# Agzs/BlockMaze

Hardware: AMD Instinct MI355X
Metric: Groth16 proofs/sec (send circuit, alt_bn128) (higher is better)
Workload: dtype u32 limbs (254-bit Fq/Fr Montgomery; all MSM accumulations, the H query's weighted bucket sum and the transforms' tiles on nine 29-bit limbs)

## Files before the change

### __graft_entry__.py

```python
import os, subprocess, sys

ROOT = os.path.dirname(os.path.abspath(__file__))
if ROOT not in sys.path:
    sys.path.insert(0, ROOT)

def build():
    subprocess.check_call(["make", "-C", os.path.join(ROOT, "blockmaze_amd", "csrc"), "-j8"])
    subprocess.check_call(["make", "-s", "-C", os.path.join(ROOT, "blockmaze_amd", "csrc"), "-j8", "tsan"])
    subprocess.check_call(["make", "-C", os.path.join(ROOT, "oracle"), "oracle"])
    if os.path.isdir("/root/reference/libsnark-vnt"):
        subprocess.check_call(["make", "-C", os.path.join(ROOT, "oracle"), "-j8", "ref"])
    import blockmaze_amd
    from blockmaze_amd import engine
    engine.lib()

def smoke():
    import numpy as np
    sys.path.insert(0, os.path.join(ROOT, "tests"))
    from blockmaze_amd import engine as e
    from oracle import pyoracle as o
    from r1cs_util import random_r1cs
    e.init()
    n = 2000; g = o.SplitMix64(1); P = o.g1_consecutive(g.field(), n); K = o.to_arr([g.field() for _ in range(n)])
    got = o.g1_from(e.msm(1, P, K))[0]; assert got == o.msm_g1(P, K), "MSM mismatch vs oracle"
    cs, z = random_r1cs(3, 3, 200, 300); dev = e.R1cs(3, 200, 300, cs.rowptr, cs.col, cs.coeff)
    assert np.array_equal(dev.witness_map(z), o.witness_map(cs, z)), "witness map mismatch vs oracle"
    import json
    d = os.path.join(ROOT, "tests", "golden", "groth16_small"); meta = json.load(open(os.path.join(d, "meta.json"))); z = o.load_witness(os.path.join(d, "wit.bin"))
    p = e.Prover(os.path.join(d, "pk.txt")); proof = p.prove(z, int(meta["r"], 16), int(meta["s"], 16)); p.close()
    assert proof == meta["proof"], "proof bytes differ from the reference prover's"
    assert e.verify(os.path.join(d, "vk.txt"), proof, o.from_arr(z[:meta["n_inputs"]]))
    print("smoke ok: MSM, witness map and a Groth16 proof on", e.lib().zkgpu_version().decode(), "match the oracle")

if __name__ == "__main__":
    build()
```

### blockmaze_amd/csrc/capi_engine.cpp

```cpp
#include <cstring>
#include <memory>
#include <mutex>
#include <string>
#include <vector>
#include "../../include/zkgpu.h"
#include "gpu.hpp"

namespace zk {
void probe_field(int field, int op, const uint8_t *a, const uint8_t *b, uint8_t *out, size_t n);
void probe_fq2(int op, const uint8_t *a, const uint8_t *b, uint8_t *out, size_t n);
void probe_group(int group, int op, const uint8_t *a, const uint8_t *b, uint8_t *out, size_t n);
void probe_field29(int field, int op, const uint32_t *a, const uint32_t *b, const uint32_t *c, const uint32_t *d, uint32_t *out, size_t n);
void probe_point29(int op, const uint32_t *a, const uint32_t *b, uint32_t *out, uint32_t *flags, size_t n);
}
using namespace zk;
using namespace zk::host;

static thread_local std::string g_err;
void zkgpu_set_error(const std::string &s) { g_err = s; }
std::mutex g_gpu_mutex;

template <class Fn> static int guarded(Fn fn) {
  try { if (!gpu_available()) { g_err = "no HIP device visible; libzkgpu has no CPU fallback"; return ZKGPU_ERR_NO_DEVICE; }
        std::lock_guard<std::mutex> lk(g_gpu_mutex); return fn(); }
// ... 66 lines not shown
    }
    else {
      std::vector<G2AffineRaw> raw(n ? n : 1);
      for (size_t i = 0; i < n; i++) g2_to_raw(points + 128 * i, raw[i]);
      m->g2.reset(new MsmG2(raw.data(), n, c, (filter_ones & 1) != 0, true, (filter_ones & 2) != 0));
    }
    m->scalars = DevBuf<Fe32>(n ? n : 1); h = m.release(); return ZKGPU_OK; });
  return rc == ZKGPU_OK ? h : nullptr;
}
int zkgpu_msm_set_scalars(zkgpu_msm *h, const uint8_t *scalars, size_t n) { return guarded([&] { if (!h || n != h->n) { g_err = "scalar count";
    return ZKGPU_ERR_ARG; }
  if (n) { h->scalars.upload((const Fe32 *)scalars, n); fr_to_mont_dev(h->scalars.get(), n); gpu_sync(); } return ZKGPU_OK; }); }
int zkgpu_msm_run(zkgpu_msm *h, uint8_t *out) { return guarded([&] { if (!h) return ZKGPU_ERR_ARG;
  if (h->group == 1) { h->g1->run(h->scalars.get(), nullptr); g1_out(h->g1->result(), out); } else { h->g2->run(h->scalars.get(), nullptr);
      g2_out(h->g2->result(), out); } return ZKGPU_OK; }); }
void zkgpu_msm_destroy(zkgpu_msm *h) { guarded([&] { delete h; return ZKGPU_OK; }); }
static int msm_oneshot(int group, const uint8_t *points, const uint8_t *scalars, size_t n, int c, int fo, uint8_t *out) {
  zkgpu_msm *h = zkgpu_msm_create(group, points, n, c, fo);
  if (!h) return ZKGPU_ERR_RUNTIME;
  int rc = zkgpu_msm_set_scalars(h, scalars, n);
  if (rc == ZKGPU_OK) rc = zkgpu_msm_run(h, out);
  zkgpu_msm_destroy(h);
  return rc;
}
int zkgpu_msm_g1(const uint8_t *points, const uint8_t *scalars, size_t n, int c, int fo, uint8_t out[64]) {
  return msm_oneshot(1, points, scalars, n, c, fo, out);
}
int zkgpu_msm_g2(const uint8_t *points, const uint8_t *scalars, size_t n, int c, int fo, uint8_t out[128]) {
  return msm_oneshot(2, points, scalars, n, c, fo, out);
}

size_t zkgpu_domain_size(size_t min_size) {
  if (min_size <= 1) return 0; size_t lg = 0; while (((size_t)1 << lg) < min_size) lg++; if (min_size == ((size_t)1 << lg)) return lg <= 28 ? min_size : 0;
  size_t big = (size_t)1 << (lg - 1), small = min_size - big, rs = 1;
  while (rs < small) rs <<= 1;
  size_t m = (small == rs) ? min_size : big + rs;
  return lg <= 28 ? m : 0;
}
int zkgpu_domain_transform(size_t min_size, int op, uint8_t *data) { return guarded([&] { Domain d(min_size); size_t m = d.m(); DevBuf<Fe32> buf(m);
    buf.upload((const Fe32 *)data, m); fr_to_mont_dev(buf.get(), m);
  switch (op) {
    case 0: d.fft(buf.get(), 1, m);
    break;
    case 1: d.ifft(buf.get(), 1, m);
    break;
    case 2: d.coset_fft(buf.get(), 1, m);
    break;
    case 3: d.icoset_fft(buf.get(), 1, m);
    break;
    default: g_err = "op";
    return ZKGPU_ERR_ARG;
  }
  fr_from_mont_dev(buf.get(), m); buf.download((Fe32 *)data, m); return ZKGPU_OK; }); }

struct zkgpu_r1cs { R1csHost host; std::unique_ptr<R1csDev> dev; std::unique_ptr<Domain> dom; };
zkgpu_r1cs *zkgpu_r1cs_create(size_t n_inputs, size_t n_vars, size_t n_cons, const uint32_t *const rowptr[3], const uint32_t *const col[3],
    const uint8_t *const coeff[3]) {
  zkgpu_r1cs *out = nullptr;
  guarded([&] { std::unique_ptr<zkgpu_r1cs> h(new zkgpu_r1cs); h->host.n_inputs = n_inputs; h->host.n_vars = n_vars; h->host.n_cons = n_cons;
    for (int m = 0; m < 3; m++) {
      size_t nnz = rowptr[m][n_cons];
      h->host.rowptr[m].assign(rowptr[m], rowptr[m] + n_cons + 1);
      h->host.col[m].assign(col[m], col[m] + nnz);
      h->host.coeff[m].resize(nnz);
      if (nnz) memcpy(h->host.coeff[m].data(), coeff[m], 32 * nnz);
    }
    h->dev.reset(new R1csDev(h->host)); h->dom.reset(new Domain(n_cons + n_inputs + 1)); out = h.release(); return ZKGPU_OK; });
  return out;
}
void zkgpu_r1cs_destroy(zkgpu_r1cs *cs) { guarded([&] { delete cs; return ZKGPU_OK; }); }
int zkgpu_witness_map(zkgpu_r1cs *cs, const uint8_t *z, uint8_t *h_out) { return guarded([&] { if (!cs) return ZKGPU_ERR_ARG;
  size_t m = cs->dom->m(), nv = cs->host.n_vars; std::vector<Fe32> zz(nv + 1); memset(&zz[0], 0, 32); zz[0].l[0] = 1; if (nv) memcpy(&zz[1], z, 32 * nv);
  DevBuf<Fe32> zd(nv + 1), abc(3 * m); zd.upload(zz.data(), nv + 1); fr_to_mont_dev(zd.get(), nv + 1);
  cs->dev->eval(zd.get(), abc.get(), m);
  if (!cs->dev->satisfied(abc.get(), m)) {
    g_err = "assignment does not satisfy the constraint system";
    return ZKGPU_ERR_UNSATISFIED;
  }
  cs->dom->ifft(abc.get(), 3, m);
  cs->dom->coset_fft(abc.get(), 3, m);
  cs->dom->qap_pointwise(abc.get(), abc.get() + m, abc.get() + 2 * m);
  cs->dom->icoset_fft(abc.get(), 1, m);
  fr_from_mont_dev(abc.get(), m); abc.download((Fe32 *)h_out, m); memset(h_out + 32 * m, 0, 32); return ZKGPU_OK; }); }
}
```

### blockmaze_amd/csrc/gpu.hip

```cpp
#include <hip/hip_runtime.h>
#include <cstdio>
#include <cstdlib>
#include <chrono>
#include <cstring>
#include <map>
#include <vector>
#include <algorithm>
#include <mutex>
#include <atomic>
#include <mutex>
#include "gpu_internal.hpp"
#include "ntt.cuh"
#include "ecntt.cuh"

__attribute__((constructor(101))) static void zkgpu_load_time_environment() { setenv("GPU_MAX_HW_QUEUES", "16", 0); }

namespace zk {

constexpr int MAX_LANES_PER_DEVICE = 31, MAX_LANES = 1 + 8 * 28;
static uint8_t g_lane_claimed[MAX_LANES];
static std::atomic<GpuContext *> g_lanes[MAX_LANES];
static std::atomic<int> g_lane_slot[MAX_LANES];
static std::mutex g_lane_mutex;
static thread_local int t_lane = 0;
// ... 639 lines not shown
  if (cs.n_vars > cs.n_inputs) dl.upload(L, cs.n_vars - cs.n_inputs);
  DevBuf<uint8_t> b0(m * sizeof(XYZZ<Fq>)), b1(m * sizeof(XYZZ<Fq>)); XYZZ<Fq> *X = (XYZZ<Fq> *)b0.get(), *Y = (XYZZ<Fq> *)b1.get();
  auto stages = [&](XYZZ<Fq> *x, const Fe32 *tw, int lg) {
    for (int st = lg; st >= 1; st--) hipLaunchKernelGGL(k_ecntt_stage, dim3(cdiv(((size_t)1 << lg) / 2, 64)), dim3(64), 0, s, x, (const Fr *)tw, lg, st);
  };
  auto columns = [&](const XYZZ<Fq> *U, int lg) { hipLaunchKernelGGL(k_fold_c_columns, dim3(cdiv(n_all, 64)), dim3(64), 0, s, d_colptr.get(), d_rowidx.get(),
      d_kind.get(), (const Fr *)d_coef.get(), U, lg,
                     (const Affine<Fq> *)dl.get(), (uint32_t)cs.n_inputs, (uint32_t)n_all, (Affine<Fq> *)dout.get()); };
  if (!d.step) {
    HFr zinv; { Fe32 z; d.zinv.download(&z, 1); memcpy(zinv.l, &z, 32); } Fr fz; memcpy(&fz, zinv.l, 32);
    std::vector<Fe32> gm = geometric_table(m, HFr::from_u64(m).inv(), fr_coset_gen());
    DevBuf<Fe32> d_gm(m);
    d_gm.upload(gm.data(), m);
    hipLaunchKernelGGL(k_ecntt_scale_const, dim3(cdiv(m, 64)), dim3(64), 0, s, (const Affine<Fq> *)dp.get(), fz, (uint32_t)m, X);
    stages(X, d.big->tw.get(), logm);
    hipLaunchKernelGGL(k_ecntt_permute_scale, dim3(cdiv(m, 64)), dim3(64), 0, s, (const XYZZ<Fq> *)X, (const Fr *)d_gm.get(), logm, Y);
    stages(Y, d.big->itw.get(), logm);
    columns(Y, logm);
  } else {
    const int lb = d.big->logn, ls = d.small->logn;
    hipLaunchKernelGGL(k_ecntt_scale_table, dim3(cdiv(m, 64)), dim3(64), 0, s, (const Affine<Fq> *)dp.get(), (const Fr *)d.zinv.get(), (uint32_t)m, X);
    stages(X, d.big->tw.get(), lb);
    stages(X + d.B, d.small->tw.get(), ls);
    hipLaunchKernelGGL(k_ecntt_step_fwd_T, dim3(cdiv(d.B, 64)), dim3(64), 0, s, (const XYZZ<Fq> *)X, (const XYZZ<Fq> *)(X + d.B), lb, ls,
        (const Fr *)d.wpow.get(), (const Fr *)d.coset_fwd.get(), Y);
    HFr ib = HFr::from_u64(d.B).inv(), is = HFr::from_u64(d.S).inv(), hib = d.half * ib, his = d.half * is;
    Fr f_hib, f_ib, f_his;
    memcpy(&f_hib, hib.l, 32);
    memcpy(&f_ib, ib.l, 32);
    memcpy(&f_his, his.l, 32);
    hipLaunchKernelGGL(k_ecntt_step_pre, dim3(cdiv(m, 64)), dim3(64), 0, s, (const XYZZ<Fq> *)Y, X, (const Fr *)d.wpow.get(), (const Fr *)d.winvpow.get(),
        f_hib, f_ib, f_his, (uint32_t)d.B, (uint32_t)d.S);
    stages(X, d.big->itw.get(), lb); stages(X + d.B, d.small->itw.get(), ls);
    hipLaunchKernelGGL(k_ecntt_unpermute, dim3(cdiv(d.B, 64)), dim3(64), 0, s, (const XYZZ<Fq> *)X, lb, Y);
    hipLaunchKernelGGL(k_ecntt_unpermute, dim3(cdiv(d.S, 64)), dim3(64), 0, s, (const XYZZ<Fq> *)(X + d.B), ls, Y + d.B);
    columns(Y, 0);
  }
  HIP_CHECK(hipGetLastError()); dout.download(out, n_all);
}
const Fe32 *Domain::zinv_dev() const { return impl->zinv.get(); }
bool Domain::zinv_is_table() const { return impl->step; }
void Domain::qap_pointwise(Fe32 *a, const Fe32 *b, const Fe32 *c) {
  hipLaunchKernelGGL(k_qap_pointwise, dim3(cdiv(impl->m, 256)), dim3(256), 0, gpu().stream, (Fr *)a, (const Fr *)b, (const Fr *)c,
      (const Fr *)impl->zinv.get(), impl->step ? 1 : 0, (uint32_t)impl->m);
}

void expand_witness_dev(const uint8_t *packed, size_t words, const Fe32 &one_value, int canon, size_t n, Fe32 *out, uint8_t *tags, uint32_t *other_vars) {
  const uint64_t *ones = (const uint64_t *)packed, *other = ones + words, *third = other + words; const size_t nbm = canon == 2 ? 3 : 2;
  const uint32_t *off = (const uint32_t *)(ones + nbm * words); const Fr *vals = (const Fr *)(packed + expand_values_offset(words, canon));
  Fr one; memcpy(&one, &one_value, 32);
  hipLaunchKernelGGL(k_expand_witness, dim3(cdiv(n, 256)), dim3(256), 0, gpu().stream, ones, other,
      canon == 0 ? (const uint64_t *)nullptr : canon == 1 ? other : third, off, vals, one, zk_with_prio(n, ZKP_EXPAND), (Fr *)out, tags, other_vars);
}
void classify_witness_dev(const Fe32 *z, size_t n, uint8_t *tags, uint32_t *other_vars, uint32_t *counters, int parity) {
  Fr one; memcpy(&one, FrParams::R1, 32);
  hipLaunchKernelGGL(k_classify_witness, dim3(cdiv(n, 256 * CLASSIFY_PER_LANE)), dim3(256), 0, gpu().stream, (const Fr *)z, one, zk_with_prio(n, ZKP_EXPAND), tags, other_vars,
      counters + (parity & 1), counters + ((parity & 1) ^ 1));
}
void expand_board_dev(const uint8_t *board_tags, size_t n, const uint32_t *cand, const Fe32 *cand_vals, size_t n_cand, Fe32 *z, uint8_t *tags, uint32_t *other_vars,
    uint32_t *counters, int parity, bool vals_by_var) {
  Fr one; memcpy(&one, FrParams::R1, 32); const unsigned tb = cdiv(n, 256);
  hipLaunchKernelGGL(k_expand_board, dim3(tb + cdiv(n_cand, 256)), dim3(256), 0, gpu().stream, board_tags, zk_with_prio(n, ZKP_EXPAND), tb, cand, (const Fr *)cand_vals,
      (uint32_t)n_cand | (vals_by_var ? 0x80000000u : 0u), one, (Fr *)z, tags, other_vars, counters + (parity & 1), counters + ((parity & 1) ^ 1));
}
void *gpu_host_register(void *p, size_t bytes) {
  if (!p || !bytes) return nullptr; gpu();
  if (hipHostRegister(p, bytes, hipHostRegisterPortable | hipHostRegisterMapped) != hipSuccess) { (void)hipGetLastError(); return nullptr; }
  void *d = nullptr; if (hipHostGetDevicePointer(&d, p, 0) != hipSuccess || !d) { (void)hipGetLastError(); hipHostUnregister(p); return nullptr; }
  return d;
}
void gpu_host_unregister(void *p) { if (p) { (void)hipHostUnregister(p); (void)hipGetLastError(); } }
static std::atomic<uint64_t> g_general_path_repeats{0}, g_queries_without_tables{0};
uint64_t queries_without_tables() { return g_queries_without_tables.load(std::memory_order_relaxed); }
void note_query_without_tables() { g_queries_without_tables.fetch_add(1, std::memory_order_relaxed); }
uint64_t general_path_repeats() { return g_general_path_repeats.load(std::memory_order_relaxed); }
void note_general_path_repeat() { g_general_path_repeats.fetch_add(1, std::memory_order_relaxed); }
void merge_equal_columns_dev(Fe32 *z, uint8_t *tags, const uint32_t *grp_ptr, const uint32_t *grp_mem, size_t n_groups) {
  if (n_groups) hipLaunchKernelGGL(k_merge_equal_columns, dim3(cdiv(n_groups, 64)), dim3(64), 0, gpu().stream, (Fr *)z, tags, grp_ptr, grp_mem, (uint32_t)n_groups);
}
void fr_to_mont_dev(Fe32 *a, size_t n) { if (n) hipLaunchKernelGGL(k_fr_to_mont, dim3(cdiv(n, 256)), dim3(256), 0, gpu().stream, (Fr *)a, (uint32_t)n); }
void fr_from_mont_dev(Fe32 *a, size_t n) { if (n) hipLaunchKernelGGL(k_fr_from_mont, dim3(cdiv(n, 256)), dim3(256), 0, gpu().stream, (Fr *)a, (uint32_t)n); }

struct R1csArrays { size_t n_inputs, n_vars, n_cons; DevBuf<uint32_t> rowptr[3], col[3], cid[3], long_rows[3]; size_t n_long[3] = {0, 0, 0}; DevBuf<Fe32> ctab;
    DevBuf<uint32_t> long_any; size_t n_long_any = 0; };
struct R1csDev::Impl {
  std::shared_ptr<R1csArrays> a;
  size_t &n_inputs, &n_vars, &n_cons;
  DevBuf<uint32_t> (&rowptr)[3], (&col)[3], (&cid)[3], (&long_rows)[3];
  size_t (&n_long)[3];
  DevBuf<Fe32> &ctab;
  DevBuf<uint32_t> &long_any;
  size_t &n_long_any;
  DevBuf<uint32_t> flag;
  uint32_t *h_flag = nullptr;
  uint32_t *h_fail = nullptr, *d_fail = nullptr, seq = 0;
  explicit Impl(std::shared_ptr<R1csArrays> aa) : a(aa), n_inputs(a->n_inputs), n_vars(a->n_vars), n_cons(a->n_cons), rowptr(a->rowptr), col(a->col),
      cid(a->cid), long_rows(a->long_rows), n_long(a->n_long), ctab(a->ctab), long_any(a->long_any), n_long_any(a->n_long_any) {
  }
  void own_words() {
    flag = DevBuf<uint32_t>(1);
    HIP_CHECK(hipHostMalloc((void **)&h_flag, 4));
    HIP_CHECK(hipHostMalloc((void **)&h_fail, 8, hipHostMallocMapped));
    h_fail[0] = 0; h_fail[1] = 0;
    HIP_CHECK(hipHostGetDevicePointer((void **)&d_fail, h_fail, 0));
  }
  ~Impl() { if (h_flag) hipHostFree(h_flag); if (h_fail) hipHostFree(h_fail); }
};
R1csDev::R1csDev(const R1csDev &peer) : impl(new Impl(peer.impl->a)) { impl->own_words(); }
R1csDev::R1csDev(const R1csHost &h) : impl(new Impl(std::make_shared<R1csArrays>())) {
  Impl &d = *impl; d.n_inputs = h.n_inputs; d.n_vars = h.n_vars; d.n_cons = h.n_cons;
  std::vector<Fe32> tab(2); { HFr one = HFr::one(), m1 = one.neg(); memcpy(&tab[0], one.l, 32); memcpy(&tab[1], m1.l, 32); }
  struct Key { uint32_t l[8]; bool operator<(const Key &o) const { return memcmp(l, o.l, 32) < 0; } };
  std::vector<std::pair<Key, uint32_t>> seen;
  size_t cap = 1 << 12; std::vector<int64_t> slots(cap, -1); std::vector<Fe32> keys; std::vector<uint32_t> vals;
  auto lookup = [&](const Fe32 &c) -> uint32_t {
    uint64_t hsh = ((uint64_t)c.l[1] << 32 | c.l[0]) * 0x9E3779B97F4A7C15ull ^ c.l[7]; size_t pos = hsh & (cap - 1);
    for (;;) { int64_t s = slots[pos]; if (s < 0) break; if (!memcmp(&keys[s], &c, 32)) return vals[s]; pos = (pos + 1) & (cap - 1); }
    if (keys.size() * 2 >= cap) throw GpuError("r1cs: more than 2048 distinct coefficients");
    HFr v; memcpy(v.l, &c, 32); v = v.to_mont(); Fe32 m; memcpy(&m, v.l, 32); uint32_t id;
    if (!memcmp(&m, &tab[0], 32)) id = 0; else if (!memcmp(&m, &tab[1], 32)) id = 1; else { id = (uint32_t)tab.size(); tab.push_back(m); }
    slots[pos] = (int64_t)keys.size(); keys.push_back(c); vals.push_back(id); return id; };
  for (int m = 0; m < 3; m++) {
    if (h.rowptr[m].size() != h.n_cons + 1) throw GpuError("r1cs: rowptr size");
    std::vector<uint32_t> ids(h.col[m].size()); for (size_t k = 0; k < ids.size(); k++) ids[k] = lookup(h.coeff[m][k]);
    d.rowptr[m] = DevBuf<uint32_t>(h.n_cons + 1); d.rowptr[m].upload(h.rowptr[m].data(), h.n_cons + 1);
    d.col[m] = DevBuf<uint32_t>(ids.size() + 1); d.cid[m] = DevBuf<uint32_t>(ids.size() + 1);
    if (!ids.empty()) { d.col[m].upload(h.col[m].data(), ids.size()); d.cid[m].upload(ids.data(), ids.size()); }
    std::vector<uint32_t> lr; for (size_t i = 0; i < h.n_cons; i++) if (h.rowptr[m][i + 1] - h.rowptr[m][i] > R1CS_LONG_ROW) lr.push_back((uint32_t)i);
    d.n_long[m] = lr.size(); d.long_rows[m] = DevBuf<uint32_t>(lr.size() + 1); if (!lr.empty()) d.long_rows[m].upload(lr.data(), lr.size());
  }
  {
    std::vector<uint32_t> lr;
    for (size_t i = 0; i < h.n_cons; i++) {
      bool lg = false;
      for (int m = 0; m < 3; m++) lg |= h.rowptr[m][i + 1] - h.rowptr[m][i] > R1CS_LONG_ROW;
      if (lg) lr.push_back((uint32_t)i);
    }
    d.n_long_any = lr.size(); d.long_any = DevBuf<uint32_t>(lr.size() + 1); if (!lr.empty()) d.long_any.upload(lr.data(), lr.size()); }
  d.ctab = DevBuf<Fe32>(tab.size()); d.ctab.upload(tab.data(), tab.size()); d.own_words();
}
R1csDev::~R1csDev() = default;
void R1csDev::eval(const Fe32 *z, Fe32 *abc, size_t m, const uint8_t *tags, bool write_c) {
  Stage st("r1cs.rows"); Impl &d = *impl; hipStream_t s = gpu().stream; if (m < d.n_cons + d.n_inputs + 1) throw GpuError("r1cs: domain too small");
  R1csMatrices M; for (int mm = 0; mm < 3; mm++) { M.rowptr[mm] = d.rowptr[mm].get(); M.col[mm] = d.col[mm].get(); M.cid[mm] = d.cid[mm].get(); }
  if (++d.seq == 0) d.seq = 1;
  if (tags) {
    const uint32_t sb = (uint32_t)cdiv(m, 256);
    hipLaunchKernelGGL(k_r1cs_rows_tagged, dim3(sb + (unsigned)cdiv(d.n_long_any, 4)), dim3(256), 0, s, M, (const Fr *)d.ctab.get(), (const Fr *)z, tags,
        (uint32_t)d.n_cons, zk_with_prio(d.n_inputs, ZKP_ROWS), (uint32_t)m,
                       (const uint32_t *)d.long_any.get(), (uint32_t)d.n_long_any, sb, write_c ? 1 : 0, (Fr *)abc, d.seq, d.d_fail);
    return; }
  if (d.n_long_any) {
    const uint32_t sb = (uint32_t)cdiv(m, 256);
    hipLaunchKernelGGL(k_r1cs_rows_all, dim3(sb + (unsigned)cdiv(d.n_long_any, 4)), dim3(256), 0, s, M, (const Fr *)d.ctab.get(), (const Fr *)z,
        (uint32_t)d.n_cons, (uint32_t)d.n_inputs, (uint32_t)m, (const uint32_t *)d.long_any.get(), (uint32_t)d.n_long_any, sb, (Fr *)abc, d.seq, d.d_fail);
    return; }
  hipLaunchKernelGGL(k_r1cs_rows3, dim3(cdiv(m, 256)), dim3(256), 0, s, M, (const Fr *)d.ctab.get(), (const Fr *)z, (uint32_t)d.n_cons, (uint32_t)d.n_inputs,
      (uint32_t)m, (Fr *)abc, d.seq, d.d_fail);
  if (d.n_long_any) hipLaunchKernelGGL(k_r1cs_long_rows3, dim3((unsigned)d.n_long_any), dim3(64), 0, s, d.long_any.get(), M, (const Fr *)d.ctab.get(),
      (const Fr *)z, (uint32_t)m, (Fr *)abc, d.seq, d.d_fail);
}
bool R1csDev::check_result() const { return *impl->h_fail != impl->seq; }
uint32_t R1csDev::failed_row() const { return impl->h_fail[1]; }
bool R1csDev::satisfied(const Fe32 *abc, size_t m) {
  Impl &d = *impl; hipStream_t s = gpu().stream; d.flag.zero();
  if (d.n_cons) hipLaunchKernelGGL(k_r1cs_check, dim3(cdiv(d.n_cons, 256)), dim3(256), 0, s, (const Fr *)abc, (const Fr *)(abc + m), (const Fr *)(abc + 2 * m),
      (uint32_t)d.n_cons, d.flag.get());
  HIP_CHECK(hipMemcpyAsync(d.h_flag, d.flag.get(), 4, hipMemcpyDeviceToHost, s)); HIP_CHECK(hipStreamSynchronize(s)); return *d.h_flag == 0;
}

}
```

### blockmaze_amd/csrc/gpu.hpp

```cpp
#pragma once
#include <cstddef>
#include <cstdint>
#include <memory>
#include <stdexcept>
#include <string>
#include <vector>
#include "hostmath.hpp"
#include "pairing_host.hpp"

namespace zk {

struct GpuError : std::runtime_error { using std::runtime_error::runtime_error; };
struct GpuOutOfMemory : GpuError { using GpuError::GpuError; };
uint64_t queries_without_tables();
void note_query_without_tables();

struct Fe32 { uint32_t l[8]; };
struct G1AffineRaw { Fe32 x, y; };
struct G2AffineRaw { Fe32 x0, x1, y0, y1; };

class GpuContext;
GpuContext &gpu();
int gpu_device_numa_node(int device);
bool gpu_available();
// ... 109 lines not shown
  struct Snapshot { uint64_t index = 0, size = 0; uint8_t root[32]; std::vector<uint8_t> path ; std::vector<bool> index_bits; };
  explicit CommitmentTree(int depth);
  ~CommitmentTree();
  int depth() const; uint64_t size() const;
  bool append(const uint8_t *leaves, size_t n);
  void root(uint8_t out[32]);
  bool path(uint64_t index, uint8_t *siblings );
  bool find(const uint8_t leaf[32], uint64_t &index);
  bool snapshot(const uint8_t leaf[32], Snapshot &out);
  uint64_t launches() const;
  bool roots_at(const uint64_t *sizes, size_t q, uint8_t *out );
  bool match_roots(const uint64_t *sizes, size_t m, const uint8_t *rts, size_t q, bool hash_order, int32_t *match_out);
  bool match_roots_window(const uint64_t *sizes, size_t m, const uint8_t *rts, size_t q, const uint32_t *lo, const uint32_t *hi, bool hash_order, int32_t *match_out);
  bool paths_at(uint64_t size, const uint64_t *indices, size_t q, uint8_t *siblings , uint8_t *root );
  bool find_at(uint64_t size, const uint8_t leaf[32], uint64_t &index);
  bool snapshot_at(uint64_t size, const uint8_t leaf[32], Snapshot &out);
  bool rewind(uint64_t size);
  uint64_t state_launches() const;
  struct Impl; std::unique_ptr<Impl> impl;
};

class SpentSet {
 public:
  explicit SpentSet(const uint8_t *exempt , int log2_slots = 0 , const uint64_t *seed = nullptr );
  ~SpentSet();
  uint64_t size() const;
  bool exempt_key(uint8_t out[20]) const;
  bool spend(const uint8_t *keys, const uint8_t *mask, size_t n, bool commit, uint8_t *conflict, uint64_t *size_out );
  bool spend_pairs(const uint8_t *keys, const uint8_t *nkeys, size_t n, bool commit, uint8_t *conflict, uint64_t *size_out );
  void set_round_cap(uint32_t rounds);
  static void rounds(uint64_t &rounds, uint64_t &host_finishes);
  bool query(uint64_t size, const uint8_t *keys, size_t q, uint64_t *index, bool current = false);
  bool rewind(uint64_t size);
  bool read_log(uint64_t first, uint64_t count, uint8_t *out);
  void table(std::vector<uint32_t> &slots, uint64_t &seed, uint64_t &tombstones);
  static uint64_t launches();
  struct Impl; std::unique_ptr<Impl> impl;
};

void snset_pairs_finish_host(const uint8_t *keys, const uint8_t *active, size_t n, uint8_t *status, uint8_t *code);

void record_digests_dev(const uint8_t *recs, size_t n, const uint32_t mid[32], uint32_t kinds, uint8_t *out20);
uint64_t record_digest_launches();
class ProofCache {
 public:
  explicit ProofCache(uint64_t capacity , const uint8_t *salt = nullptr );
  ~ProofCache();
  const uint8_t *salt() const;
  void lookup(const uint8_t *keys, size_t q, uint8_t *hit);
  void insert(const uint8_t *keys, const uint8_t *mask, size_t n);
  void clear();
  void stats(uint64_t out[4]);
  struct Impl; std::unique_ptr<Impl> impl;
};

struct LeafRange { uint64_t first, count; };
void list_roots_dev(int depth, const uint8_t *leaves, size_t n_leaves, const LeafRange *lists, size_t n_lists, bool hash_order, uint8_t *roots);
uint64_t list_roots_launches();

struct R1csHost;
class Domain {
 public:
  explicit Domain(size_t min_size); explicit Domain(const Domain &peer); ~Domain();
  size_t m() const; bool is_step() const;
  void fft(Fe32 *data, int batch, size_t stride); void ifft(Fe32 *data, int batch, size_t stride);
  void coset_fft(Fe32 *data, int batch, size_t stride); void icoset_fft(Fe32 *data, int batch, size_t stride);
  void ifft_then_coset_fft(Fe32 *data, int batch, size_t stride);
 private: void fft_with_factors(Fe32 *data, int batch, size_t stride, const Fe32 *factors); public:
  bool supports_h_lagrange() const; void h_query_to_coset_lagrange(const G1AffineRaw *h, size_t n_in, G1AffineRaw *out );
  bool supports_c_fold() const;
  void fold_c_into_l(const G1AffineRaw *h_lagrange , const R1csHost &cs, const G1AffineRaw *L , G1AffineRaw *out);
  const Fe32 *zinv_dev() const; bool zinv_is_table() const;
  void qap_pointwise(Fe32 *a, const Fe32 *b, const Fe32 *c);
  struct Impl; std::unique_ptr<Impl> impl;
};

struct R1csHost {
  size_t n_inputs = 0, n_vars = 0, n_cons = 0;
  std::vector<uint32_t> rowptr[3], col[3]; std::vector<Fe32> coeff[3];
};
class R1csDev {
 public:
  explicit R1csDev(const R1csHost &h); explicit R1csDev(const R1csDev &peer); ~R1csDev();
  void eval(const Fe32 *z_dev, Fe32 *abc, size_t m, const uint8_t *tags_dev = nullptr, bool write_c = true);
  bool satisfied(const Fe32 *abc, size_t m);
  bool check_result() const;
  uint32_t failed_row() const;
  struct Impl; std::unique_ptr<Impl> impl;
};

void fr_to_mont_dev(Fe32 *a, size_t n); void fr_from_mont_dev(Fe32 *a, size_t n);
inline size_t expand_values_offset(size_t words, int canon) { return (((canon == 2 ? 28 : 20) * words + 31) / 32) * 32; }
void expand_witness_dev(const uint8_t *packed_dev, size_t words, const Fe32 &one_value, int canon, size_t n, Fe32 *out, uint8_t *tags_out = nullptr,
    uint32_t *other_vars_out = nullptr);
void expand_board_dev(const uint8_t *board_tags, size_t n, const uint32_t *cand, const Fe32 *cand_vals, size_t n_cand, Fe32 *z, uint8_t *tags, uint32_t *other_vars,
    uint32_t *counters, int parity, bool vals_by_var = false);
void merge_equal_columns_dev(Fe32 *z, uint8_t *tags, const uint32_t *grp_ptr, const uint32_t *grp_mem, size_t n_groups);
void classify_witness_dev(const Fe32 *z, size_t n, uint8_t *tags_out, uint32_t *other_vars_out, uint32_t *counters, int parity);

void decompress_g1(const Fe32 *xs, const uint8_t *flags, size_t n, G1AffineRaw *out);
void decompress_g2(const Fe32 *xs , const uint8_t *flags, size_t n, G2AffineRaw *out);
void fixed_base_mul_g1(const host::HG1 &base, const Fe32 *scalars, size_t n, G1AffineRaw *out);
void fixed_base_mul_g2(const host::HG2 &base, const Fe32 *scalars, size_t n, G2AffineRaw *out);
void *gpu_host_register(void *p, size_t bytes);
void gpu_host_unregister(void *p);
void gpu_sync();
void gpu_fork_aux();
void gpu_fork_one(int aux);
void gpu_fork_record();
void gpu_fork_wait(int aux);
void gpu_join_aux();
bool profiling_enabled();
uint64_t general_path_repeats();
void note_general_path_repeat();
void profile_enable(bool on); std::string profile_report();
void profile_add_host(const char *name, double ms);
struct HostSpan { const char *name; bool on; double t0; explicit HostSpan(const char *n); ~HostSpan(); HostSpan(const HostSpan &) = delete; };

}
```

### blockmaze_amd/csrc/ntt.cuh

```cuda
#pragma once
#include <hip/hip_runtime.h>
#include "field.cuh"
#include "field29.cuh"

namespace zk {

constexpr int NTT_LOCAL_LOG = 10;
constexpr int NTT_LOCAL_THREADS = 512;

__device__ __forceinline__ uint32_t bitrev32(uint32_t x, int bits) { return __brev(x) >> (32 - bits); }

__global__ void k_ntt_bitrev_scale(const Fr *__restrict__ in, Fr *__restrict__ out, const Fr *__restrict__ scale, int logn, size_t stride_in,
    size_t stride_out) {
  uint32_t i = blockIdx.x * blockDim.x + threadIdx.x, n = 1u << logn; if (i >= n) return;
  const Fr *src = in + blockIdx.y * stride_in; Fr *dst = out + blockIdx.y * stride_out; uint32_t r = bitrev32(i, logn);
  Fr v = src[r]; if (scale) v = v * scale[r]; dst[i] = v;
}

__global__ void __launch_bounds__(NTT_LOCAL_THREADS) k_ntt_local(Fr *__restrict__ data, const Fr *__restrict__ tw, int logn, int L, size_t stride) {
  extern __shared__ uint32_t lds_raw[]; Fr *tile = reinterpret_cast<Fr *>(lds_raw);
  const uint32_t T = 1u << L, half_n = 1u << (logn - 1); Fr *d = data + blockIdx.y * stride + (size_t)blockIdx.x * T;
  for (uint32_t i = threadIdx.x; i < T; i += blockDim.x) tile[i] = d[i];
  __syncthreads();
  for (int s = 1; s <= L; s++) {
    const uint32_t half = 1u << (s - 1);
    for (uint32_t b = threadIdx.x; b < T / 2; b += blockDim.x) {
      uint32_t j = b & (half - 1), k = (b >> (s - 1)) << s, i0 = k + j, i1 = i0 + half;
      Fr t = tile[i1]; if (j) t = t * tw[j * (half_n >> (s - 1))];
      Fr u = tile[i0]; tile[i0] = u + t; tile[i1] = u - t;
    }
    __syncthreads();
  }
  for (uint32_t i = threadIdx.x; i < T; i += blockDim.x) d[i] = tile[i];
}

__global__ void k_ntt_stage(Fr *__restrict__ data, const Fr *__restrict__ tw, int logn, int s, size_t stride) {
  uint32_t b = blockIdx.x * blockDim.x + threadIdx.x, half_n = 1u << (logn - 1); if (b >= half_n) return;
  Fr *d = data + blockIdx.y * stride; const uint32_t half = 1u << (s - 1); uint32_t j = b & (half - 1), i0 = ((b >> (s - 1)) << s) + j, i1 = i0 + half;
  Fr t = d[i1]; if (j) t = t * tw[j * (half_n >> (s - 1))];
  Fr u = d[i0]; d[i0] = u + t; d[i1] = u - t;
}

constexpr int NTT_TILE_LOG = 11;
constexpr int NTT_TILE_THREADS = 256;

__device__ __forceinline__ uint32_t ntt_pad(uint32_t e) { return e + (e >> 4); }
__device__ __forceinline__ Fr29 ntt29_from_words(const Fr &v) { uint32_t w[8];
#pragma unroll
  for (int i = 0; i < 8; i++) w[i] = v.l[i];
  return Fr29::unpack(w); }
__device__ __forceinline__ Fr ntt29_to_words(const Fr29 &t) { uint32_t w[8]; t.pack_words(w); Fr r;
#pragma unroll
  for (int i = 0; i < 8; i++) r.l[i] = w[i];
  return Fr::reduce_once(r); }
template <int R> __device__ __forceinline__ void ntt29_lds_pass(Fr29 *tile, const Fr29 *twl, int logN, int logC, int s) {
  const uint32_t groups = (1u << (logN - R)) << logC, cmask = (1u << logC) - 1; const int sh = s - R;
  for (uint32_t w = threadIdx.x; w < groups; w += blockDim.x) {
    const uint32_t g = w >> logC, c = w & cmask, base = ((g >> sh) << s) | (g & ((1u << sh) - 1)); Fr29 x[1 << R];
#pragma unroll
    for (int q = 0; q < (1 << R); q++) x[q] = tile[ntt_pad(((base + ((uint32_t)q << sh)) << logC) + c)];
#pragma unroll
    for (int t = 0; t < R; t++) {
      const int st = s - t, hx = 1 << (R - 1 - t), bits = logN - st;
#pragma unroll
      for (int q = 0; q < (1 << R); q++) if (!(q & hx)) {
        const uint32_t blk = (base + ((uint32_t)q << sh)) >> st; Fr29 u = x[q], v = x[q + hx];
        if (bits) v = Fr29::mul(v, twl[(__brev(blk) >> (32 - bits)) << (st - 1)]);
        const Fr29 sum = Fr29::add_raw(u, v), dif = Fr29::sub_product(u, v);
        const bool carry_now = (t & 1) == 1 || t == R - 1;
        x[q] = carry_now ? sum.norm() : sum;
        x[q + hx] = carry_now ? dif.norm() : dif;
      }
    }
#pragma unroll
    for (int q = 0; q < (1 << R); q++) tile[ntt_pad(((base + ((uint32_t)q << sh)) << logC) + c)] = x[q];
  }
  __syncthreads();
}
__device__ __forceinline__ void ntt29_lds_transform(Fr29 *tile, Fr29 *twl, int logN, int logC, const Fr *__restrict__ tw261, uint32_t tws, int radix_log) {
  for (uint32_t j = threadIdx.x; j < (1u << logN) / 2; j += blockDim.x) twl[j] = ntt29_from_words(tw261[j * tws]);
  __syncthreads();
  int s = logN;
  if (radix_log >= 3) for (; s >= 3; s -= 3) ntt29_lds_pass<3>(tile, twl, logN, logC, s);
  if (radix_log >= 2) for (; s >= 2; s -= 2) ntt29_lds_pass<2>(tile, twl, logN, logC, s);
  for (; s >= 1; s -= 1) ntt29_lds_pass<1>(tile, twl, logN, logC, s);
}
// ... 249 lines not shown
  uint32_t col[3][R1CS_HEAD], cid[3][R1CS_HEAD];
#pragma unroll
  for (int mm = 0; mm < 3; mm++) {
#pragma unroll
    for (int j = 0; j < R1CS_HEAD; j++) {
      const bool valid = beg[mm] + j < end[mm];
      col[mm][j] = valid ? M.col[mm][beg[mm] + j] : 0u;
      cid[mm][j] = valid ? M.cid[mm][beg[mm] + j] : 0u;
    }
  }
  uint8_t tag[3][R1CS_HEAD];
#pragma unroll
  for (int mm = 0; mm < 3; mm++) {
#pragma unroll
    for (int j = 0; j < R1CS_HEAD; j++) tag[mm][j] = beg[mm] + j < end[mm] ? tags[col[mm][j]] : ZTAG_ZERO;
  }
#pragma unroll
  for (int mm = 0; mm < 3; mm++) {
    Fr acc = Fr::zero();
#pragma unroll
    for (int j = 0; j < R1CS_HEAD; j++) {
      if (tag[mm][j] == ZTAG_ZERO) continue;
      const Fr coef = ctab[cid[mm][j]];
      if (tag[mm][j] == ZTAG_ONE) { acc = acc + coef; continue; }
      const Fr v = z[col[mm][j]];
      if (cid[mm][j] == 0) acc = acc + v;
      else if (cid[mm][j] == 1) acc = acc - v;
      else acc = acc + coef * v;
    }
    for (uint32_t k = beg[mm] + R1CS_HEAD; k < end[mm]; k++) acc = r1cs_term_tagged(acc, M.cid[mm][k], M.col[mm][k], ctab, z, tags);
    out[mm] = acc;
  }
}
__global__ void __launch_bounds__(256) k_r1cs_rows_tagged(R1csMatrices M, const Fr *__restrict__ ctab, const Fr *__restrict__ z,
    const uint8_t *__restrict__ tags, uint32_t n_rows, uint32_t n_inputs, uint32_t m,
                                                          const uint32_t *__restrict__ long_rows, uint32_t n_long, uint32_t short_blocks, int write_c,
                                                              Fr *__restrict__ abc, uint32_t seq, uint32_t *fail) {
  zk_take_prio(n_inputs);
  if (blockIdx.x < short_blocks) {
    const uint32_t r = blockIdx.x * blockDim.x + threadIdx.x;
    if (r >= m) return;
    if (r >= n_rows) {
      abc[r] = r <= n_rows + n_inputs ? z[r - n_rows] : Fr::zero();
      abc[m + r] = Fr::zero();
      if (write_c) abc[2 * (size_t)m + r] = Fr::zero();
      return;
    }
    if (M.rowptr[0][r + 1] - M.rowptr[0][r] > R1CS_LONG_ROW || M.rowptr[1][r + 1] - M.rowptr[1][r] > R1CS_LONG_ROW || M.rowptr[2][r + 1] -
        M.rowptr[2][r] > R1CS_LONG_ROW) return;
    Fr v[3];
    r1cs_rows_tagged_lane(M, r, ctab, z, tags, v);
    abc[r] = v[0];
    abc[m + r] = v[1];
    if (write_c) abc[2 * (size_t)m + r] = v[2];
    if (v[0] * v[1] != v[2]) { fail[1] = r; *fail = seq; }
    return;
  }
  const uint32_t w = (blockIdx.x - short_blocks) * 4 + (threadIdx.x >> 6), lane = threadIdx.x & 63;
  if (w >= n_long) return;
  const uint32_t r = long_rows[w];
  Fr v[3];
#pragma unroll
  for (int mm = 0; mm < 3; mm++) {
    Fr acc = Fr::zero();
    const uint32_t *col = M.col[mm], *cid = M.cid[mm];
    for (uint32_t k = M.rowptr[mm][r] + lane, e = M.rowptr[mm][r + 1]; k < e; k += 64) acc = r1cs_term_tagged(acc, cid[k], col[k], ctab, z, tags);
    const uint32_t len = M.rowptr[mm][r + 1] - M.rowptr[mm][r];
#pragma unroll 1
    for (int d = 32; d >= 1; d >>= 1) {
      if ((uint32_t)d >= len) continue;
      Fr o;
      for (int i = 0; i < 8; i++) o.l[i] = __shfl_down(acc.l[i], d, 64);
      acc = acc + o;
    }
    v[mm] = acc;
  }
  if (lane == 0) {
    abc[r] = v[0];
    abc[m + r] = v[1];
    if (write_c) abc[2 * (size_t)m + r] = v[2];
    if (v[0] * v[1] != v[2]) { fail[1] = r; *fail = seq; }
  }
}
__global__ void k_r1cs_check(const Fr *__restrict__ a, const Fr *__restrict__ b, const Fr *__restrict__ c, uint32_t n_rows, uint32_t *flag) {
  uint32_t r = blockIdx.x * blockDim.x + threadIdx.x; if (r >= n_rows) return; if (a[r] * b[r] != c[r]) atomicOr(flag, 1u);
}

}
```

Measured before the change: 1341.

## Evaluate short R1CS rows from a sliced column-major packed term layout

Adds a host-built sliced ELL-style layout in which each 64-row slice stores its terms column-major, with column and coefficient id packed into one word. A new kernel has each lane evaluate one row by reading coalesced packed terms and prefetching tags, in place of the CSR layout with its separate col and cid arrays. Long rows still go through the wavefront CSR path. The goal is fewer and better-coalesced index loads in the witness-row evaluation, at the cost of extra device memory for padding, a build step at setup, and a new test hook that can force the CSR path.

```diff
diff --git a/__graft_entry__.py b/__graft_entry__.py
--- a/__graft_entry__.py
+++ b/__graft_entry__.py
@@ -7,6 +7,7 @@
 def build():
     subprocess.check_call(["make", "-C", os.path.join(ROOT, "blockmaze_amd", "csrc"), "-j8"])
     subprocess.check_call(["make", "-s", "-C", os.path.join(ROOT, "blockmaze_amd", "csrc"), "-j8", "tsan"])
+    subprocess.check_call(["make", "-s", "-C", os.path.join(ROOT, "blockmaze_amd", "csrc"), "-j8", "hooks"])
     subprocess.check_call(["make", "-C", os.path.join(ROOT, "oracle"), "oracle"])
     if os.path.isdir("/root/reference/libsnark-vnt"):
         subprocess.check_call(["make", "-C", os.path.join(ROOT, "oracle"), "-j8", "ref"])
diff --git a/blockmaze_amd/csrc/capi_engine.cpp b/blockmaze_amd/csrc/capi_engine.cpp
--- a/blockmaze_amd/csrc/capi_engine.cpp
+++ b/blockmaze_amd/csrc/capi_engine.cpp
@@ -172,4 +172,15 @@
   cs->dom->qap_pointwise(abc.get(), abc.get() + m, abc.get() + 2 * m);
   cs->dom->icoset_fft(abc.get(), 1, m);
   fr_from_mont_dev(abc.get(), m); abc.download((Fe32 *)h_out, m); memset(h_out + 32 * m, 0, 32); return ZKGPU_OK; }); }
+#ifdef ZKGPU_TEST_HOOKS
+int zkgpu_test_r1cs_rows(zkgpu_r1cs *cs, const uint8_t *z, int mode, uint8_t *abc_out, uint64_t info[4]) { return guarded([&] {
+  if (!cs || !abc_out || !info || mode < 0 || mode > 2) return ZKGPU_ERR_ARG;
+  const size_t m = cs->dom->m(), nv = cs->host.n_vars, n = nv + 1; std::vector<Fe32> zz(n); memset(&zz[0], 0, 32); zz[0].l[0] = 1; if (nv) memcpy(&zz[1], z, 32 * nv);
+  DevBuf<Fe32> zd(n), abc(3 * m); zd.upload(zz.data(), n); fr_to_mont_dev(zd.get(), n); abc.zero();
+  DevBuf<uint8_t> tags(n); DevBuf<uint32_t> other(n), counters(2); counters.zero();
+  if (mode) classify_witness_dev(zd.get(), n, tags.get(), other.get(), counters.get(), 0);
+  cs->dev->eval(zd.get(), abc.get(), m, mode ? tags.get() : nullptr, true, mode == 2); gpu_sync();
+  info[0] = cs->dev->check_result() ? 1 : 0; info[1] = info[0] ? 0 : cs->dev->failed_row(); info[2] = cs->dev->sliced() ? 1 : 0; info[3] = cs->dev->sliced_bytes();
+  abc.download((Fe32 *)abc_out, 3 * m); return ZKGPU_OK; }); }
+#endif
 }
diff --git a/blockmaze_amd/csrc/gpu.hip b/blockmaze_amd/csrc/gpu.hip
--- a/blockmaze_amd/csrc/gpu.hip
+++ b/blockmaze_amd/csrc/gpu.hip
@@ -745,7 +745,8 @@
 void fr_from_mont_dev(Fe32 *a, size_t n) { if (n) hipLaunchKernelGGL(k_fr_from_mont, dim3(cdiv(n, 256)), dim3(256), 0, gpu().stream, (Fr *)a, (uint32_t)n); }
 
 struct R1csArrays { size_t n_inputs, n_vars, n_cons; DevBuf<uint32_t> rowptr[3], col[3], cid[3], long_rows[3]; size_t n_long[3] = {0, 0, 0}; DevBuf<Fe32> ctab;
-    DevBuf<uint32_t> long_any; size_t n_long_any = 0; };
+    DevBuf<uint32_t> long_any; size_t n_long_any = 0;
+    bool sliced = false; DevBuf<uint32_t> slice_hdr, slice_terms; size_t sliced_bytes = 0; };
 struct R1csDev::Impl {
   std::shared_ptr<R1csArrays> a;
   size_t &n_inputs, &n_vars, &n_cons;
@@ -783,9 +784,10 @@
     HFr v; memcpy(v.l, &c, 32); v = v.to_mont(); Fe32 m; memcpy(&m, v.l, 32); uint32_t id;
     if (!memcmp(&m, &tab[0], 32)) id = 0; else if (!memcmp(&m, &tab[1], 32)) id = 1; else { id = (uint32_t)tab.size(); tab.push_back(m); }
     slots[pos] = (int64_t)keys.size(); keys.push_back(c); vals.push_back(id); return id; };
+  std::vector<uint32_t> cids[3];
   for (int m = 0; m < 3; m++) {
     if (h.rowptr[m].size() != h.n_cons + 1) throw GpuError("r1cs: rowptr size");
-    std::vector<uint32_t> ids(h.col[m].size()); for (size_t k = 0; k < ids.size(); k++) ids[k] = lookup(h.coeff[m][k]);
+    std::vector<uint32_t> &ids = cids[m]; ids.resize(h.col[m].size()); for (size_t k = 0; k < ids.size(); k++) ids[k] = lookup(h.coeff[m][k]);
     d.rowptr[m] = DevBuf<uint32_t>(h.n_cons + 1); d.rowptr[m].upload(h.rowptr[m].data(), h.n_cons + 1);
     d.col[m] = DevBuf<uint32_t>(ids.size() + 1); d.cid[m] = DevBuf<uint32_t>(ids.size() + 1);
     if (!ids.empty()) { d.col[m].upload(h.col[m].data(), ids.size()); d.cid[m].upload(ids.data(), ids.size()); }
@@ -800,15 +802,32 @@
       if (lg) lr.push_back((uint32_t)i);
     }
     d.n_long_any = lr.size(); d.long_any = DevBuf<uint32_t>(lr.size() + 1); if (!lr.empty()) d.long_any.upload(lr.data(), lr.size()); }
-  d.ctab = DevBuf<Fe32>(tab.size()); d.ctab.upload(tab.data(), tab.size()); d.own_words();
-}
+  d.ctab = DevBuf<Fe32>(tab.size()); d.ctab.upload(tab.data(), tab.size());
+  {
+    const R1csSliced sl = r1cs_build_sliced(h.n_cons, h.rowptr, h.col, cids, h.n_vars + 1, tab.size(), R1CS_LONG_ROW);
+    if (sl.usable) {
+      R1csArrays &a = *d.a;
+      a.slice_hdr = DevBuf<uint32_t>(sl.hdr.size() * 8 + 8); if (!sl.hdr.empty()) a.slice_hdr.upload(reinterpret_cast<const uint32_t *>(sl.hdr.data()), sl.hdr.size() * 8);
+      a.slice_terms = DevBuf<uint32_t>(sl.terms.size()); a.slice_terms.upload(sl.terms.data(), sl.terms.size());
+      a.sliced_bytes = sl.bytes(); a.sliced = true;
+    }
+  }
+  d.own_words();
+}
+bool R1csDev::sliced() const { return impl->a->sliced; }
+size_t R1csDev::sliced_bytes() const { return impl->a->sliced_bytes; }
 R1csDev::~R1csDev() = default;
-void R1csDev::eval(const Fe32 *z, Fe32 *abc, size_t m, const uint8_t *tags, bool write_c) {
+void R1csDev::eval(const Fe32 *z, Fe32 *abc, size_t m, const uint8_t *tags, bool write_c, bool csr_only) {
   Stage st("r1cs.rows"); Impl &d = *impl; hipStream_t s = gpu().stream; if (m < d.n_cons + d.n_inputs + 1) throw GpuError("r1cs: domain too small");
   R1csMatrices M; for (int mm = 0; mm < 3; mm++) { M.rowptr[mm] = d.rowptr[mm].get(); M.col[mm] = d.col[mm].get(); M.cid[mm] = d.cid[mm].get(); }
   if (++d.seq == 0) d.seq = 1;
   if (tags) {
     const uint32_t sb = (uint32_t)cdiv(m, 256);
+    if (d.a->sliced && !csr_only) {
+      hipLaunchKernelGGL(k_r1cs_rows_sliced, dim3(sb + (unsigned)cdiv(d.n_long_any, 4)), dim3(256), 0, s, reinterpret_cast<const R1csSliceHeader *>(d.a->slice_hdr.get()),
+          (const uint32_t *)d.a->slice_terms.get(), M, (const Fr *)d.ctab.get(), (const Fr *)z, tags, (uint32_t)d.n_cons, zk_with_prio(d.n_inputs, ZKP_ROWS), (uint32_t)m,
+          (const uint32_t *)d.long_any.get(), (uint32_t)d.n_long_any, sb, write_c ? 1 : 0, (Fr *)abc, d.seq, d.d_fail);
+      return; }
     hipLaunchKernelGGL(k_r1cs_rows_tagged, dim3(sb + (unsigned)cdiv(d.n_long_any, 4)), dim3(256), 0, s, M, (const Fr *)d.ctab.get(), (const Fr *)z, tags,
         (uint32_t)d.n_cons, zk_with_prio(d.n_inputs, ZKP_ROWS), (uint32_t)m,
                        (const uint32_t *)d.long_any.get(), (uint32_t)d.n_long_any, sb, write_c ? 1 : 0, (Fr *)abc, d.seq, d.d_fail);
diff --git a/blockmaze_amd/csrc/gpu.hpp b/blockmaze_amd/csrc/gpu.hpp
--- a/blockmaze_amd/csrc/gpu.hpp
+++ b/blockmaze_amd/csrc/gpu.hpp
@@ -215,7 +215,8 @@
 class R1csDev {
  public:
   explicit R1csDev(const R1csHost &h); explicit R1csDev(const R1csDev &peer); ~R1csDev();
-  void eval(const Fe32 *z_dev, Fe32 *abc, size_t m, const uint8_t *tags_dev = nullptr, bool write_c = true);
+  void eval(const Fe32 *z_dev, Fe32 *abc, size_t m, const uint8_t *tags_dev = nullptr, bool write_c = true, bool csr_only = false);
+  bool sliced() const; size_t sliced_bytes() const;
   bool satisfied(const Fe32 *abc, size_t m);
   bool check_result() const;
   uint32_t failed_row() const;
diff --git a/blockmaze_amd/csrc/ntt.cuh b/blockmaze_amd/csrc/ntt.cuh
--- a/blockmaze_amd/csrc/ntt.cuh
+++ b/blockmaze_amd/csrc/ntt.cuh
@@ -2,6 +2,7 @@
 #include <hip/hip_runtime.h>
 #include "field.cuh"
 #include "field29.cuh"
+#include "r1cs_sliced.hpp"
 
 namespace zk {
 
@@ -417,6 +418,102 @@
     if (v[0] * v[1] != v[2]) { fail[1] = r; *fail = seq; }
   }
 }
+__device__ __forceinline__ void r1cs_sliced_chunk(Fr &acc, const uint32_t (&t)[R1CS_HEAD], const uint8_t (&tag)[R1CS_HEAD], const Fr *__restrict__ ctab,
+    const Fr *__restrict__ z) {
+#pragma unroll
+  for (int j = 0; j < R1CS_HEAD; j++) {
+    if (tag[j] == ZTAG_ZERO) continue;
+    const uint32_t col = t[j] & R1CS_COL_MASK, ci = t[j] >> R1CS_COL_BITS;
+    const Fr coef = ctab[ci];
+    if (tag[j] == ZTAG_ONE) { acc = acc + coef; continue; }
+    const Fr v = z[col];
+    if (ci == 0) acc = acc + v;
+    else if (ci == 1) acc = acc - v;
+    else acc = acc + coef * v;
+  }
+}
+__device__ __forceinline__ Fr r1cs_sliced_matrix(uint32_t base, uint32_t width, const uint32_t (&t)[R1CS_HEAD], const uint8_t (&tag)[R1CS_HEAD],
+    const uint32_t *__restrict__ terms, uint32_t lane, const Fr *__restrict__ ctab, const Fr *__restrict__ z, const uint8_t *__restrict__ tags) {
+  Fr acc = Fr::zero();
+  r1cs_sliced_chunk(acc, t, tag, ctab, z);
+  for (uint32_t j0 = R1CS_HEAD; j0 < width; j0 += R1CS_HEAD) {
+    uint32_t u[R1CS_HEAD]; uint8_t ug[R1CS_HEAD];
+#pragma unroll
+    for (int j = 0; j < R1CS_HEAD; j++) u[j] = j0 + j < width ? terms[base + (j0 + j) * R1CS_SLICE_ROWS + lane] : R1CS_NO_TERM;
+#pragma unroll
+    for (int j = 0; j < R1CS_HEAD; j++) ug[j] = u[j] != R1CS_NO_TERM ? tags[u[j] & R1CS_COL_MASK] : ZTAG_ZERO;
+    r1cs_sliced_chunk(acc, u, ug, ctab, z);
+  }
+  return acc;
+}
+__device__ __forceinline__ void r1cs_rows_sliced_lane(const R1csSliceHeader &h, const uint32_t *__restrict__ terms, uint32_t lane, const Fr *__restrict__ ctab,
+    const Fr *__restrict__ z, const uint8_t *__restrict__ tags, Fr (&out)[3]) {
+  uint32_t t[3][R1CS_HEAD];
+#pragma unroll
+  for (int mm = 0; mm < 3; mm++) {
+#pragma unroll
+    for (int j = 0; j < R1CS_HEAD; j++) t[mm][j] = (uint32_t)j < h.width[mm] ? terms[h.base[mm] + (uint32_t)j * R1CS_SLICE_ROWS + lane] : R1CS_NO_TERM;
+  }
+  uint8_t tag[3][R1CS_HEAD];
+#pragma unroll
+  for (int mm = 0; mm < 3; mm++) {
+#pragma unroll
+    for (int j = 0; j < R1CS_HEAD; j++) tag[mm][j] = t[mm][j] != R1CS_NO_TERM ? tags[t[mm][j] & R1CS_COL_MASK] : ZTAG_ZERO;
+  }
+  out[0] = r1cs_sliced_matrix(h.base[0], h.width[0], t[0], tag[0], terms, lane, ctab, z, tags);
+  out[1] = r1cs_sliced_matrix(h.base[1], h.width[1], t[1], tag[1], terms, lane, ctab, z, tags);
+  out[2] = r1cs_sliced_matrix(h.base[2], h.width[2], t[2], tag[2], terms, lane, ctab, z, tags);
+}
+__global__ void __launch_bounds__(256) k_r1cs_rows_sliced(const R1csSliceHeader *__restrict__ hdr, const uint32_t *__restrict__ terms, R1csMatrices M,
+    const Fr *__restrict__ ctab, const Fr *__restrict__ z, const uint8_t *__restrict__ tags, uint32_t n_rows, uint32_t n_inputs, uint32_t m,
+    const uint32_t *__restrict__ long_rows, uint32_t n_long, uint32_t short_blocks, int write_c, Fr *__restrict__ abc, uint32_t seq, uint32_t *fail) {
+  zk_take_prio(n_inputs);
+  if (blockIdx.x < short_blocks) {
+    const uint32_t r = blockIdx.x * blockDim.x + threadIdx.x;
+    if (r >= m) return;
+    if (r >= n_rows) {
+      abc[r] = r <= n_rows + n_inputs ? z[r - n_rows] : Fr::zero();
+      abc[m + r] = Fr::zero();
+      if (write_c) abc[2 * (size_t)m + r] = Fr::zero();
+      return;
+    }
+    const uint32_t lane = threadIdx.x & 63;
+    const R1csSliceHeader h = hdr[__builtin_amdgcn_readfirstlane(r >> 6)];
+    if (((lane < 32 ? h.long_lo >> lane : h.long_hi >> (lane - 32)) & 1u) != 0) return;
+    Fr v[3];
+    r1cs_rows_sliced_lane(h, terms, lane, ctab, z, tags, v);
+    abc[r] = v[0];
+    abc[m + r] = v[1];
+    if (write_c) abc[2 * (size_t)m + r] = v[2];
+    if (v[0] * v[1] != v[2]) { fail[1] = r; *fail = seq; }
+    return;
+  }
+  const uint32_t w = (blockIdx.x - short_blocks) * 4 + (threadIdx.x >> 6), lane = threadIdx.x & 63;
+  if (w >= n_long) return;
+  const uint32_t r = long_rows[w];
+  Fr v[3];
+#pragma unroll
+  for (int mm = 0; mm < 3; mm++) {
+    Fr acc = Fr::zero();
+    const uint32_t *col = M.col[mm], *cid = M.cid[mm];
+    for (uint32_t k = M.rowptr[mm][r] + lane, e = M.rowptr[mm][r + 1]; k < e; k += 64) acc = r1cs_term_tagged(acc, cid[k], col[k], ctab, z, tags);
+    const uint32_t len = M.rowptr[mm][r + 1] - M.rowptr[mm][r];
+#pragma unroll 1
+    for (int d = 32; d >= 1; d >>= 1) {
+      if ((uint32_t)d >= len) continue;
+      Fr o;
+      for (int i = 0; i < 8; i++) o.l[i] = __shfl_down(acc.l[i], d, 64);
+      acc = acc + o;
+    }
+    v[mm] = acc;
+  }
+  if (lane == 0) {
+    abc[r] = v[0];
+    abc[m + r] = v[1];
+    if (write_c) abc[2 * (size_t)m + r] = v[2];
+    if (v[0] * v[1] != v[2]) { fail[1] = r; *fail = seq; }
+  }
+}
 __global__ void k_r1cs_check(const Fr *__restrict__ a, const Fr *__restrict__ b, const Fr *__restrict__ c, uint32_t n_rows, uint32_t *flag) {
   uint32_t r = blockIdx.x * blockDim.x + threadIdx.x; if (r >= n_rows) return; if (a[r] * b[r] != c[r]) atomicOr(flag, 1u);
 }
diff --git a/blockmaze_amd/csrc/r1cs_sliced.hpp b/blockmaze_amd/csrc/r1cs_sliced.hpp
--- /dev/null
+++ b/blockmaze_amd/csrc/r1cs_sliced.hpp
@@ -0,0 +1,56 @@
+#pragma once
+#include <cstddef>
+#include <cstdint>
+#include <vector>
+
+namespace zk {
+
+constexpr uint32_t R1CS_SLICE_ROWS = 64, R1CS_COL_BITS = 21, R1CS_CID_BITS = 11, R1CS_COL_MASK = (1u << R1CS_COL_BITS) - 1, R1CS_NO_TERM = 0xffffffffu;
+struct R1csSliceHeader { uint32_t base[3], width[3], long_lo, long_hi; };
+static_assert(sizeof(R1csSliceHeader) == 32, "eight words a slice");
+struct R1csSliced { bool usable = false; std::vector<R1csSliceHeader> hdr; std::vector<uint32_t> terms;
+  size_t bytes() const { return hdr.size() * sizeof(R1csSliceHeader) + terms.size() * sizeof(uint32_t); } };
+
+inline bool r1cs_sliced_fits(size_t n_columns, size_t n_coeffs) { return n_columns < ((size_t)1 << R1CS_COL_BITS) && n_coeffs <= ((size_t)1 << R1CS_CID_BITS); }
+
+inline R1csSliced r1cs_build_sliced(size_t n_cons, const std::vector<uint32_t> (&rowptr)[3], const std::vector<uint32_t> (&col)[3],
+    const std::vector<uint32_t> (&cid)[3], size_t n_columns, size_t n_coeffs, uint32_t long_row) {
+  R1csSliced s;
+  if (!r1cs_sliced_fits(n_columns, n_coeffs)) return s;
+  for (int m = 0; m < 3; m++) {
+    if (rowptr[m].size() != n_cons + 1 || col[m].size() < rowptr[m][n_cons] || cid[m].size() < rowptr[m][n_cons]) return s;
+    for (size_t k = 0; k < rowptr[m][n_cons]; k++) if (col[m][k] >= n_columns || cid[m][k] >= n_coeffs) return s;
+  }
+  const size_t n_slices = (n_cons + R1CS_SLICE_ROWS - 1) / R1CS_SLICE_ROWS;
+  auto len = [&](int m, size_t r) { return rowptr[m][r + 1] - rowptr[m][r]; };
+  auto is_long = [&](size_t r) { return len(0, r) > long_row || len(1, r) > long_row || len(2, r) > long_row; };
+  s.hdr.resize(n_slices);
+  size_t total = 0;
+  for (size_t sl = 0; sl < n_slices; sl++) {
+    R1csSliceHeader &h = s.hdr[sl]; h = R1csSliceHeader{};
+    const size_t r0 = sl * R1CS_SLICE_ROWS, r1 = r0 + R1CS_SLICE_ROWS < n_cons ? r0 + R1CS_SLICE_ROWS : n_cons;
+    for (size_t r = r0; r < r1; r++) {
+      if (is_long(r)) { const uint32_t l = (uint32_t)(r - r0); if (l < 32) h.long_lo |= 1u << l; else h.long_hi |= 1u << (l - 32); continue; }
+      for (int m = 0; m < 3; m++) if (len(m, r) > h.width[m]) h.width[m] = len(m, r);
+    }
+    for (int m = 0; m < 3; m++) {
+      if (total > 0xffffffffull) return R1csSliced{};
+      h.base[m] = (uint32_t)total; total += (size_t)h.width[m] * R1CS_SLICE_ROWS;
+    }
+  }
+  if (total > 0xffffffffull) return R1csSliced{};
+  s.terms.assign(total ? total : 1, R1CS_NO_TERM);
+  for (size_t sl = 0; sl < n_slices; sl++) {
+    const R1csSliceHeader &h = s.hdr[sl];
+    const size_t r0 = sl * R1CS_SLICE_ROWS, r1 = r0 + R1CS_SLICE_ROWS < n_cons ? r0 + R1CS_SLICE_ROWS : n_cons;
+    for (size_t r = r0; r < r1; r++) {
+      if (is_long(r)) continue;
+      for (int m = 0; m < 3; m++)
+        for (uint32_t j = 0, k = rowptr[m][r]; k < rowptr[m][r + 1]; j++, k++) s.terms[(size_t)h.base[m] + (size_t)j * R1CS_SLICE_ROWS + (r - r0)] = col[m][k] | cid[m][k] << R1CS_COL_BITS;
+    }
+  }
+  s.usable = true;
+  return s;
+}
+
+}
```

Measured after the change: 1341. No clear change (-0.1%).
